# akanazawa/human_dynamics

Measured on AMD Instinct MI355X. Metric: frames/sec/GPU (ResNet+temporal+SMPL, 224x224); SMPL verts max-abs-err, higher is better.
Workload: dtype f16x3

## Files before the change

### human_dynamics_amd/_lib.py

```python
from __future__ import annotations

import ctypes as C
import os

from . import devflags

HERE = os.path.dirname(os.path.abspath(__file__))
LIB_PATH = devflags.get("LIB_PATH") or os.path.join(HERE, "libhmmr_hip.so")

HMMR_F32, HMMR_BF16, HMMR_F16X3 = 0, 1, 2
FLAG_SATURATED = 1
FLAG_NAN = 2
ABI_VERSION = 19
RESNET_UNITS = 16
RESNET_PROF_SLOTS = 64
MAX_TEMPORAL_BLOCKS = 8
MAX_REGRESSORS = 8

_vp, _fp, _ip = C.c_void_p, C.c_void_p, C.c_void_p


class ConvDesc(C.Structure):
    _fields_ = [
        ("in_", _vp), ("w", _vp), ("scale", _fp), ("shift", _fp), ("res", _vp), ("out", _vp),
        ("out2", _vp), ("scale2", _fp), ("shift2", _fp),
        ("in_dtype", C.c_int), ("out_dtype", C.c_int),
        ("n_img", C.c_int), ("hin", C.c_int), ("win", C.c_int), ("cin", C.c_int),
        ("in_img_stride", C.c_int64), ("in_row_stride", C.c_int), ("in_px_stride", C.c_int),
        ("kh", C.c_int), ("kw", C.c_int), ("sy", C.c_int), ("sx", C.c_int), ("py", C.c_int), ("px", C.c_int),
        ("ho", C.c_int), ("wo", C.c_int), ("cout", C.c_int), ("ldo", C.c_int),
        ("ldr", C.c_int), ("res_strided", C.c_int), ("res_img_stride", C.c_int64),
        ("res_row_stride", C.c_int), ("res_px_stride", C.c_int),
        ("relu", C.c_int), ("tile", C.c_int),
        ("split_k", C.c_int), ("ws", _vp), ("ws_bytes", C.c_size_t),
        ("pro_scale", _fp), ("pro_shift", _fp),
        ("out_b", _vp), ("ldo_b", C.c_int), ("n_split", C.c_int), ("relu_b", C.c_int),
        ("in2", _vp), ("cin2", C.c_int), ("k_order", C.c_int),
        ("batch", C.c_int), ("batch_in_bytes", C.c_int64), ("batch_w_bytes", C.c_int64), ("batch_out_bytes", C.c_int64),
        ("batch_res_bytes", C.c_int64), ("batch_scale_bytes", C.c_int64), ("batch_shift_bytes", C.c_int64),
    ]


class TailDesc(C.Structure):
    _fields_ = [
        ("dtype", C.c_int), ("h2", _vp), ("m", C.c_int), ("c_mid", C.c_int), ("depth", C.c_int),
        ("w3", _vp), ("scale3", _fp), ("shift3", _fp),
        ("res", _vp), ("ldr", C.c_int), ("res_strided", C.c_int), ("res_img_stride", C.c_int64),
        ("res_row_stride", C.c_int), ("res_px_stride", C.c_int), ("ho", C.c_int), ("wo", C.c_int),
        ("out", _vp), ("pre_scale", _fp), ("pre_shift", _fp),
        ("w1", _vp), ("scale1", _fp), ("shift1", _fp), ("relu1", C.c_int), ("n2", C.c_int),
        ("out_h1", _vp),
        ("h1", _vp), ("hin", C.c_int), ("win", C.c_int), ("w2", _vp), ("scale2", _fp), ("shift2", _fp),
        ("xp", _vp), ("wsc", _vp), ("shift_sc", _fp),
        ("conv2_stride", C.c_int), ("out_pre", _vp),
        ("pair_stream", _vp), ("c_xp", C.c_int), ("unit_stream", _vp), ("trunk_keep_stride", C.c_int),
    ]


class Debug(C.Structure):
    _fields_ = [("stem_route", C.c_int), ("stem_no_conv1", C.c_int), ("gemm_probe", C.c_int), ("smpl_blend_mfma", C.c_int), ("ief_no_group", C.c_int), ("reserved", C.c_int * 2), ("keep_dead_rows", C.c_int),
                ("pair_min_pixels", C.c_int), ("pair_two_tile_min", C.c_int), ("pair_form", C.c_int)]


class LaunchCounts(C.Structure):
    _fields_ = [("unit_pair", C.c_ulonglong), ("b1_unit", C.c_ulonglong), ("tail_split", C.c_ulonglong), ("conv3x3_stream", C.c_ulonglong),
                ("conv1x1_stream", C.c_ulonglong)]


class StemCounts(C.Structure):
    _fields_ = [(k, C.c_ulonglong) for k in ("fused", "fused_conv1", "repack", "gemm", "pool")]


TILE_GENERIC, TILE_PATCH, TILE_STREAM_3X3, TILE_STREAM_1X1 = range(4)
CONV_TILE_MAX = 63


class ConvTileInfo(C.Structure):
    _fields_ = [(k, C.c_int) for k in ("tile", "family", "fm", "fn", "wgm", "wgn", "pixels", "channels", "row_blocks", "depth", "occupancy", "wmax",
                                       "split_only", "conv3_form", "cols", "tune_cols", "narrow", "rank", "candidate")] + [("text", C.c_char_p)]


class Layer(C.Structure):
    _fields_ = [("w", _vp), ("scale", _fp), ("shift", _fp), ("tile", C.c_int), ("k_order", C.c_int)]


class ResnetUnit(C.Structure):
    _fields_ = [("conv1", Layer), ("conv2", Layer), ("conv3", Layer), ("shortcut", Layer), ("c3sc", Layer), ("sc_c1", Layer),
                ("w3_frag", _vp), ("w1n_frag", _vp), ("pair_stream", _vp), ("conv1_frag", _vp), ("unit_stream", _vp), ("pre_scale", _fp), ("pre_shift", _fp),
                ("c_in", C.c_int), ("base", C.c_int), ("depth", C.c_int), ("stride", C.c_int),
                ("fuse_preact", C.c_int), ("fuse_tail", C.c_int)]


class ResnetWeights(C.Structure):
    _fields_ = [("dtype", C.c_int), ("stem", Layer),
                ("unit", ResnetUnit * RESNET_UNITS), ("post_scale", _fp), ("post_shift", _fp)]


SC_NONE, SC_LAUNCH, SC_LAUNCH_WITH_CONV1, SC_IN_CONV3, SC_IN_TAIL = range(5)
CONV1_LAUNCH, CONV1_READY = range(2)
CONV2_LAUNCH, CONV2_IN_TAIL = range(2)
END_CONV3_LAUNCH, END_TAIL_BF16, END_TAIL_BF16_STRIDE2, END_TAIL_SPLIT, END_B1_UNIT, END_UNIT_PAIR = range(6)


class UnitPlan(C.Structure):
    _fields_ = [(k, C.c_int) for k in ("shortcut", "conv1", "conv2", "end", "reads_fused_preact", "writes_raw", "writes_pre",
                                       "pair_demoted", "swaps_t1_t2", "leaves_h1", "trunk_keep_stride")]


def resnet_plan(rw, n_total):
    plan = (UnitPlan * RESNET_UNITS)()
    check(load().hmmr_resnet50_plan(C.byref(rw), int(n_total), plan), "hmmr_resnet50_plan")
    return list(plan)


class TemporalBlock(C.Structure):
    _fields_ = [("gn1_gamma", _fp), ("gn1_beta", _fp), ("conv1", Layer),
                ("gn2_gamma", _fp), ("gn2_beta", _fp), ("conv2", Layer)]


class TemporalWeights(C.Structure):
    _fields_ = [("dtype", C.c_int), ("num_blocks", C.c_int), ("block", TemporalBlock * MAX_TEMPORAL_BLOCKS)]


class HallucinatorWeights(C.Structure):
    _fields_ = [("dtype", C.c_int), ("fc1", Layer), ("fc2", Layer), ("fc3", Layer)]


class IefRegressor(C.Structure):
    _fields_ = [("nd", C.c_int), ("fc1_phi", Layer), ("fc1_theta", Layer), ("fc2", Layer), ("fc3", Layer)]


class IefWeights(C.Structure):
    _fields_ = [("dtype", C.c_int), ("num_regressors", C.c_int), ("num_stages", C.c_int),
                ("reg", IefRegressor * MAX_REGRESSORS), ("mean_theta", _fp),
                ("no_optcam", C.c_int), ("delta_from_start", C.c_int)]


class IefRegGrads(C.Structure):
    _fields_ = [(k, _fp) for k in ("d_fc1_phi", "d_fc1_theta", "d_fc2", "d_fc3", "d_b1", "d_b2", "d_b3")]


class IefBwdDesc(C.Structure):
    _fields_ = [("strips", _fp), ("omega_start", _fp), ("keep", _vp), ("keep_scale", C.c_float), ("m", C.c_int), ("d_omegas", _fp),
                ("d_strips", _fp), ("d_omega_start", _fp), ("reg", IefRegGrads * MAX_REGRESSORS)]


TEMPORAL_GRAD_NAMES = ("gn1_gamma", "gn1_beta", "conv1", "b1", "gn2_gamma", "gn2_beta", "conv2", "b2")
HALLUCINATOR_GRAD_NAMES = ("fc1", "fc2", "fc3", "b1", "b2", "b3")


class TemporalBlockGrads(C.Structure):
    _fields_ = [("d_" + k, _fp) for k in TEMPORAL_GRAD_NAMES]


class TemporalBwdDesc(C.Structure):
    _fields_ = [("phi", _fp), ("b", C.c_int), ("t", C.c_int), ("d_strips", _fp), ("d_phi", _fp),
                ("block", TemporalBlockGrads * MAX_TEMPORAL_BLOCKS)]


class HallucinatorBwdDesc(C.Structure):
    _fields_ = [("phi", _fp), ("m", C.c_int), ("d_out", _fp), ("d_phi", _fp)] + [("d_" + k, _fp) for k in HALLUCINATOR_GRAD_NAMES]


DISC_POSE_LAYERS = ("conv1", "conv2", "heads", "fc1", "fc2", "fc_out")
DISC_POSE_GRAD_NAMES = ("conv1", "bc1", "conv2", "bc2", "heads", "bj", "fc1", "b1", "fc2", "b2", "fc_out", "bo")


class Rows(C.Structure):
    _fields_ = [("ptr", _fp), ("ld", C.c_int64), ("n", C.c_int)]


class DiscPoseWeights(C.Structure):
    _fields_ = [("dtype", C.c_int)] + [(k, Layer) for k in DISC_POSE_LAYERS]


class DiscPoseGrads(C.Structure):
    _fields_ = [("d_" + k, _fp) for k in DISC_POSE_GRAD_NAMES]


class DiscPoseBwdDesc(C.Structure):
    _fields_ = [("rows_a", Rows), ("rows_b", Rows), ("d_out", _fp), ("d_poses_a", _fp), ("ld_a", C.c_int64), ("d_poses_b", _fp),
                ("ld_b", C.c_int64), ("grads", DiscPoseGrads)]


class PosePriorDesc(C.Structure):
    _fields_ = [("real", Rows), ("fake", Rows), ("w_e", C.c_float), ("w_d", C.c_float), ("losses", _fp), ("d_rs_fake", _fp),
                ("grads", DiscPoseGrads)]


class SmplConsts(C.Structure):
    _fields_ = [("num_verts", C.c_int), ("num_kps", C.c_int), ("lbs_nnz", C.c_int), ("vpad", C.c_int),
                ("dirs", _fp), ("j_template", _fp), ("j_shapedirs", _fp), ("parents", _ip),
                ("lbs_idx", _ip), ("lbs_w", _fp), ("kreg_ptr", _ip), ("kreg_idx", _ip), ("kreg_val", _fp),
                ("dirs_split", _vp)]


class SmplGradConsts(C.Structure):
    _fields_ = [("num_verts", C.c_int), ("num_kps", C.c_int), ("vk_ptr", _ip), ("vk_idx", _ip), ("vk_val", _fp)]


LOSS_KP, LOSS_KP_OPTCAM, LOSS_JOINTS, LOSS_SMPL, LOSS_CONST, LOSS_SHAPE_PRIOR = 1, 2, 4, 8, 16, 32
LOSS_NAMES = ("e_kp", "e_joints", "e_smpl_pose", "e_smpl_shape", "e_const", "e_shape", "total")
LOSS_NO_VISIBLE, LOSS_NOT_FINITE = 1, 2


class SeqLossDesc(C.Structure):
    _fields_ = [("B", C.c_int), ("T", C.c_int), ("K", C.c_int), ("delta_t", C.c_int), ("flags", C.c_uint), ("weights", C.c_float * 6),
                ("kps_pred", _fp), ("joints_pred", _fp), ("rs_pred", _fp), ("beta_pred", _fp), ("ld_beta", C.c_int),
                ("kps_gt", _fp), ("joints_gt", _fp), ("rs_gt", _fp), ("shapes_gt", _fp), ("has_gt3d_smpl", _fp), ("has_gt3d_joints", _fp),
                ("losses", _fp), ("d_kps", _fp), ("d_joints", _fp), ("d_rs", _fp), ("d_beta", _fp), ("best_cam", _fp), ("status", _vp),
                ("ws", _vp), ("ws_bytes", C.c_size_t)]


# ... 266 lines not shown
```

### human_dynamics_amd/build.py

```python
from __future__ import annotations

import os
import subprocess
import sys
from concurrent.futures import ThreadPoolExecutor

HERE = os.path.dirname(os.path.abspath(__file__))
CSRC = os.path.join(HERE, "csrc")
INCLUDE = os.path.join(os.path.dirname(HERE), "include")
LIB = os.path.join(HERE, "libhmmr_hip.so")
SOURCES = ["api.cpp", "pack.cpp", "gemm_conv.hip", "conv3x3_stream.hip", "conv1x1_stream.hip", "stem.hip", "bottleneck.hip", "bottleneck_split.hip", "unit_pair.hip", "b1_unit.hip", "resnet.hip", "temporal.hip", "ief.hip", "ief_grad.hip", "movie_grad.hip", "disc_pose.hip", "smpl.hip", "smpl_grad.hip", "losses.hip", "adam.hip", "eval_metrics.hip", "preprocess.hip", "tube.hip", "track.hip", "handoff.hip", "render.hip", "collage.hip", "person_view.hip", "windows.hip", "video_plan.cpp", "video.cpp", "probe.hip"]
HIPCC = os.environ.get("HIPCC", "/opt/rocm/bin/hipcc")
FLAGS = ["--offload-arch=gfx950", "-O3", "-std=c++17", "-fPIC", "-fno-slp-vectorize", "-I", INCLUDE, "-I", CSRC,
         "-Wall", "-Wno-unused-function"]


EXTRA_FLAGS = {"pack.cpp": ["-ffp-contract=off"], "track.hip": ["-ffp-contract=off"], "collage.hip": ["-ffp-contract=off"],
               "tube.hip": ["-ffp-contract=off"], "person_view.hip": ["-ffp-contract=off"], "adam.hip": ["-ffp-contract=off"]}


def _newer(src, dst):
    return (not os.path.exists(dst)) or os.path.getmtime(src) > os.path.getmtime(dst)


def _deps():
    return sorted(os.path.join(d, h) for d in (CSRC, INCLUDE) for h in os.listdir(d) if h.endswith(".h"))


def build(force=False, verbose=True):
    objs, jobs = [], []
    for src in SOURCES:
        s = os.path.join(CSRC, src)
        o = os.path.join(CSRC, os.path.splitext(src)[0] + ".o")
        objs.append(o)
        if force or _newer(s, o) or any(_newer(d, o) for d in _deps()):
            lang = ["-x", "hip"] if src.endswith(".hip") else []
            jobs.append([HIPCC] + FLAGS + EXTRA_FLAGS.get(src, []) + lang + ["-c", s, "-o", o])

    def run(cmd):
        if verbose:
            print(" ".join(cmd), flush=True)
        r = subprocess.run(cmd, stdout=subprocess.PIPE, stderr=subprocess.STDOUT, text=True)
        if r.returncode != 0:
            raise RuntimeError("hipcc failed:\n%s\n%s" % (" ".join(cmd), r.stdout))
        if verbose and r.stdout.strip():
            print(r.stdout)

    if jobs:
        with ThreadPoolExecutor(max_workers=min(len(jobs), os.cpu_count() or 4)) as ex:
            list(ex.map(run, jobs))
    if jobs or force or not os.path.exists(LIB):
        run([HIPCC, "--offload-arch=gfx950", "-shared", "-fPIC", "-o", LIB] + objs)
        from . import isa_check
        unsafe = isa_check.unsafe_forms(LIB)
        if unsafe:
            os.replace(LIB, LIB + ".rejected")
            raise RuntimeError("the linked library holds packed-fp32 instructions gfx950 gets wrong beside MFMAs (isa_check.py, DESIGN 4.6); "
                               "kept as %s.rejected:\n%s" % (LIB, "\n".join("  %d x %s %s in %s" % (n, op, mods, kern)
                                                                             for (kern, op, mods), n in sorted(unsafe.items()))))
        if verbose:
            print("isa_check: %s" % ("no disassembler (%s) or no gfx950 code object found in the library: NOT checked" % isa_check.OBJDUMP if unsafe is None
                                     else "no packed-fp32 instruction reads source 1's high register into its low result"), flush=True)
    return LIB


if __name__ == "__main__":
    print(build(force="--force" in sys.argv))
```

### human_dynamics_amd/csrc/ief.hip

```cpp
#include "common.h"
#include "hmmr_hip.h"
#include "tail_sched.h"
#include "workspace.h"

template <typename TO>
__global__ void cast_rows_kernel(const float* __restrict__ in, TO* __restrict__ out, long long n8) {
    const long long i = (long long)blockIdx.x * blockDim.x + threadIdx.x;
    if (i >= n8) return;
    float v[8];
    load8(in + i * 8, v);
    store8(out + i * 8, v);
}

__global__ void ief_init_theta_kernel(const float* __restrict__ src, int ld_src, int off, int nd,
                                      float* __restrict__ theta, float* __restrict__ theta_other, int m, long long th_stride) {
    const long long i = (long long)blockIdx.x * blockDim.x + threadIdx.x;
    if (i >= (long long)m * LDT) return;
    const int row = (int)(i / LDT), col = (int)(i % LDT);
    const long long z = (long long)blockIdx.y * th_stride;
    theta[z + i] = col < nd ? src[(long long)row * ld_src + off + col] : 0.f;
    theta_other[z + i] = 0.f;
}

__global__ void ief_finalize_kernel(const float* __restrict__ theta, const float* __restrict__ bsrc, int ld_b,
                                    int mode, float* __restrict__ out, int m, long long th_stride) {
    const long long i = (long long)blockIdx.x * blockDim.x + threadIdx.x;
    if (i >= (long long)m * 85) return;
    const int row = (int)(i / 85), col = (int)(i % 85);
    theta += (long long)blockIdx.y * th_stride;
    out += (long long)blockIdx.y * m * 85;
    float v;
    if (mode == 0) v = theta[(long long)row * LDT + col];
    else if (col >= 75) v = bsrc[(long long)row * ld_b + col];
    else if (mode == 2) v = theta[(long long)row * LDT + col];
    else if (col == 0) v = 1.f;
    else if (col < 3) v = 0.f;
    else v = theta[(long long)row * LDT + (col - 3)];
    out[i] = v;
}

struct IefBufs { size_t xin, pre, h1, h2, th[2], sk, skbytes, pre_s, th_s, total; };
static IefBufs ief_layout(int m, int dtype, int group) {
    const size_t e = dtype == HMMR_BF16 ? 2 : 4;
    const size_t g = group > 1 ? group : 1;
    IefBufs b; WsCarver c;
    b.xin = c.take((size_t)m * 2048 * e);
    b.pre_s = align_up((size_t)m * 1024 * e, 256);
    b.th_s = align_up((size_t)m * LDT * 4, 256);
    b.pre = c.take(g * b.pre_s);
    b.h1 = c.take(g * b.pre_s);
    b.h2 = c.take(g * b.pre_s);
    b.th[0] = c.take(g * b.th_s);
    b.th[1] = c.take(g * b.th_s);
    b.skbytes = g * hmmr_conv_splitk_workspace_bytes(m, 1024, IEF_SPLIT_K);
    b.sk = c.take(b.skbytes);
    b.total = c.total();
    return b;
}

extern "C" size_t hmmr_ief_workspace_bytes(int m, int num_regressors, int dtype) {
    return m > 0 ? ief_layout(m, dtype, num_regressors - 1).total : 0;
}

extern "C" int hmmr_ief_fwd(const hmmr_ief_weights_t* w, const float* strips, int m, float* omegas,
                            void* ws, size_t ws_bytes, void* stream) {
    return hmmr_ief_fwd_from(w, strips, nullptr, m, omegas, ws, ws_bytes, stream);
}

extern "C" int hmmr_ief_fwd_from(const hmmr_ief_weights_t* w, const float* strips, const float* omega_start, int m,
                                 float* omegas, void* ws, size_t ws_bytes, void* stream) {
    HMMR_REQUIRE(w && strips && omegas && ws, "hmmr_ief_fwd: null argument");
    HMMR_REQUIRE(m > 0, "hmmr_ief_fwd: m must be positive");
    HMMR_REQUIRE(w->num_regressors >= 1 && w->num_regressors <= HMMR_MAX_REGRESSORS, "hmmr_ief_fwd: bad num_regressors");
    HMMR_REQUIRE(w->reg[0].nd == 85, "hmmr_ief_fwd: regressor 0 must predict 85-D omega");
    const int nd_delta = w->no_optcam ? 75 : 72;
    for (int r = 0; r < w->num_regressors; ++r)
        HMMR_REQUIRE(w->reg[r].nd == (r == 0 ? 85 : nd_delta), "hmmr_ief_fwd: regressor %d has nd=%d (expected %d)", r,
                     w->reg[r].nd, r == 0 ? 85 : nd_delta);
    const IefBufs L = ief_layout(m, w->dtype, w->num_regressors - 1);
    HMMR_REQUIRE(ws_bytes >= L.total, "hmmr_ief_fwd: workspace too small");
    hipStream_t s = (hipStream_t)stream;
    char* base = (char*)ws;
    const void* xin = strips;
    if (w->dtype != HMMR_F32) {
        const long long n8 = (long long)m * 2048 / 8;
        if (w->dtype == HMMR_BF16)
            hipLaunchKernelGGL(cast_rows_kernel<bf16_t>, dim3((unsigned)((n8 + 255) / 256)), dim3(256), 0, s, strips,
                               (bf16_t*)(base + L.xin), n8);
        else
            hipLaunchKernelGGL(cast_rows_kernel<bsplit_t>, dim3((unsigned)((n8 + 255) / 256)), dim3(256), 0, s, strips,
                               (bsplit_t*)(base + L.xin), n8);
        HMMR_CHECK_HIP(hipGetLastError());
        xin = base + L.xin;
    }
    void* pre = base + L.pre; void* h1 = base + L.h1; void* h2 = base + L.h2;
    float* th[2] = {(float*)(base + L.th[0]), (float*)(base + L.th[1])};
    const unsigned gth = (unsigned)(((long long)m * LDT + 255) / 256);
    const unsigned gfin = (unsigned)(((long long)m * 85 + 255) / 256);
    const int nd_group = w->num_regressors - 1;
    struct Strides { long long w, scale, shift; };
    auto strides_of = [&](const hmmr_layer_t hmmr_ief_regressor_t::*lay, Strides& st) -> bool {
        st = Strides{0, 0, 0};
        for (int r = 2; r < w->num_regressors; ++r) {
            const hmmr_layer_t& a = w->reg[r - 1].*lay; const hmmr_layer_t& b = w->reg[r].*lay;
            const Strides cur = {(const char*)b.w - (const char*)a.w,
                                 a.scale ? (const char*)b.scale - (const char*)a.scale : 0,
                                 a.shift ? (const char*)b.shift - (const char*)a.shift : 0};
            if (!a.scale != !b.scale || !a.shift != !b.shift) return false;
            if (r > 2 && (cur.w != st.w || cur.scale != st.scale || cur.shift != st.shift)) return false;
            st = cur;
        }
        return ((st.w | st.scale | st.shift) & 15) == 0;
    };
    Strides s_phi, s_th, s_fc2, s_fc3;
    const bool grouped = nd_group >= 2 && !hmmr_debug_state()->ief_no_group &&
                         strides_of(&hmmr_ief_regressor_t::fc1_phi, s_phi) && strides_of(&hmmr_ief_regressor_t::fc1_theta, s_th) &&
                         strides_of(&hmmr_ief_regressor_t::fc2, s_fc2) && strides_of(&hmmr_ief_regressor_t::fc3, s_fc3);
    const float* start = omega_start ? omega_start : w->mean_theta;
    const int ld_start = omega_start ? 85 : 0;
    const float* dsrc = w->delta_from_start ? start : (const float*)omegas;
    const int ld_d = w->delta_from_start ? ld_start : 85;
    auto run = [&](int r, int nb, const Strides& z_phi, const Strides& z_th, const Strides& z_fc2, const Strides& z_fc3) -> int {
        const hmmr_ief_regressor_t& R = w->reg[r];
        const long long ths = (long long)(L.th_s / 4);
        auto group = [&](hmmr_conv_desc_t& d, const Strides& z, long long in_b, long long out_b, long long res_b) {
            if (nb < 2) return;
            d.batch = nb; d.batch_in_bytes = in_b; d.batch_w_bytes = z.w; d.batch_out_bytes = out_b; d.batch_res_bytes = res_b;
            d.batch_scale_bytes = z.scale; d.batch_shift_bytes = z.shift;
        };
        if (r == 0)
            hipLaunchKernelGGL(ief_init_theta_kernel, dim3(gth), dim3(256), 0, s, start, ld_start, 0, 85, th[0], th[1], m, ths);
        else
            hipLaunchKernelGGL(ief_init_theta_kernel, dim3(gth, nb), dim3(256), 0, s, dsrc, ld_d, w->no_optcam ? 0 : 3, nd_delta,
                               th[0], th[1], m, ths);
        HMMR_CHECK_HIP(hipGetLastError());
        hmmr_conv_desc_t d = fc_desc(xin, w->dtype, m, 2048, R.fc1_phi, pre, w->dtype, 1024, 1024, IEF_SPLIT_K, base + L.sk, L.skbytes);
        group(d, z_phi, 0, (long long)L.pre_s, 0);
        if (hmmr_conv_gemm(&d, s)) return -2;
        int cur = 0;
        for (int st = 0; st < w->num_stages; ++st) {
            d = fc_desc(th[cur], HMMR_F32, m, LDT, R.fc1_theta, h1, w->dtype, 1024, 1024);
            d.res = pre; d.ldr = 1024; d.relu = 1;
            group(d, z_th, (long long)L.th_s, (long long)L.pre_s, (long long)L.pre_s);
            if (hmmr_conv_gemm(&d, s)) return -2;
            d = fc_desc(h1, w->dtype, m, 1024, R.fc2, h2, w->dtype, 1024, 1024, IEF_SPLIT_K, base + L.sk, L.skbytes);
            d.relu = 1;
            group(d, z_fc2, (long long)L.pre_s, (long long)L.pre_s, 0);
            if (hmmr_conv_gemm(&d, s)) return -2;
            d = fc_desc(h2, w->dtype, m, 1024, R.fc3, th[cur ^ 1], HMMR_F32, R.nd, LDT, IEF_SPLIT_K, base + L.sk, L.skbytes);
            d.res = th[cur]; d.ldr = LDT;
            group(d, z_fc3, (long long)L.pre_s, (long long)L.th_s, (long long)L.th_s);
            if (hmmr_conv_gemm(&d, s)) return -2;
            cur ^= 1;
        }
        hipLaunchKernelGGL(ief_finalize_kernel, dim3(gfin, nb), dim3(256), 0, s, (const float*)th[cur],
                           dsrc, ld_d, r == 0 ? 0 : (w->no_optcam ? 2 : 1), omegas + (size_t)r * m * 85, m, ths);
        HMMR_CHECK_HIP(hipGetLastError());
        return 0;
    };
    const Strides none = {0, 0, 0};
    if (run(0, 1, none, none, none, none)) return -2;
    if (grouped) return run(1, nd_group, s_phi, s_th, s_fc2, s_fc3);
    for (int r = 1; r < w->num_regressors; ++r)
        if (run(r, 1, none, none, none, none)) return -2;
    return 0;
}
```

### human_dynamics_amd/csrc/stream_kit.h

```cpp
#pragma once
#include <type_traits>
#include <utility>

#include "common.h"
#include "hmmr_hip.h"

template <class K, class... Args>
static int launch_with_lds(K kern, DeviceOnce& once, dim3 grid, dim3 block, int lds_attr, int lds, hipStream_t stream, Args... args) {
    if (const unsigned long long bit = once.due()) {
        HMMR_CHECK_HIP(hipFuncSetAttribute((const void*)kern, hipFuncAttributeMaxDynamicSharedMemorySize, lds_attr));
        once.mark(bit);
    }
    hipLaunchKernelGGL(kern, grid, block, lds, stream, args...);
    HMMR_CHECK_HIP(hipGetLastError());
    return 0;
}
static inline unsigned long long* probe_stamp_buffer() {
    const hmmr_debug_t* d = hmmr_debug_state();
    return (unsigned long long*)(((unsigned long long)(unsigned)d->reserved[1] << 32) | (unsigned)d->reserved[0]);
}

struct xfrag { shalf8 hi, lo; };
template <int V> using ic = std::integral_constant<int, V>;
template <class F, int... I> __device__ __forceinline__ void static_for(F&& f, std::integer_sequence<int, I...>) { (f(ic<I>{}), ...); }

typedef const __attribute__((address_space(1))) void* gptr_t;
typedef __attribute__((address_space(3))) void* lptr_t;
__device__ __forceinline__ unsigned lds_addr(void* p) { return (unsigned)(unsigned long long)(lptr_t)p; }

constexpr unsigned waitcnt_imm(int vm, int lgkm) { return (vm & 15) | (7 << 4) | (lgkm << 8) | ((vm >> 4) << 14); }
static_assert(waitcnt_imm(63, 0) == (63 | (7 << 4) | (0 << 8) | (3 << 14)) && waitcnt_imm(63, 0) == 0xC07F, "lgkmcnt(0) alone: the literal five files spelled out");
static_assert(waitcnt_imm(0, 0) == 0x0070 && waitcnt_imm(63, 15) == 0xCF7F, "everything; nothing");
static_assert(waitcnt_imm(63, 5) == 0xC57F && waitcnt_imm(37, 0) == 0x8075 && waitcnt_imm(37, 15) == 0x8F75, "lgkmcnt(5) alone; vmcnt(37) lgkmcnt(0); vmcnt(37) alone");
template <int N> __device__ __forceinline__ void wait_vm_lgkm0() {
    static_assert(N >= 0 && N < 64, "vmcnt is a 6-bit counter");
    __builtin_amdgcn_s_waitcnt(waitcnt_imm(N, 0));
}
template <int N> __device__ __forceinline__ void wait_vm() {
    static_assert(N >= 0 && N < 64, "vmcnt is a 6-bit counter");
    __builtin_amdgcn_s_waitcnt(waitcnt_imm(N, 15));
}
template <int N> __device__ __forceinline__ void wait_lgkm() {
    static_assert(N >= 0 && N <= 15, "lgkmcnt is a 4-bit counter");
    __builtin_amdgcn_s_waitcnt(waitcnt_imm(63, N));
}

template <class T, int OFF> __device__ __forceinline__ T lds_rd128(unsigned addr) {
    static_assert(sizeof(T) == 16, "a ds_read_b128");
    T v; asm volatile("ds_read_b128 %0, %1 offset:%2" : "=v"(v) : "v"(addr), "n"(OFF)); return v;
}
template <int OFF> __device__ __forceinline__ unsigned long long lds_rd64(unsigned addr) {
    unsigned long long v; asm volatile("ds_read_b64 %0, %1 offset:%2" : "=v"(v) : "v"(addr), "n"(OFF)); return v;
}
template <int OFF> __device__ __forceinline__ void lds_wr64(unsigned addr, unsigned long long v) {
    asm volatile("ds_write_b64 %0, %1 offset:%2" : : "v"(addr), "v"(v), "n"(OFF) : "memory");
}

static __device__ u32x4 g_dump_page[64 + 32] __attribute__((unused));

#ifndef TRUNK_DEAD_SHARED_PAGE
#define TRUNK_DEAD_SHARED_PAGE 0
#endif
constexpr int TRUNK_DEAD_WGS = 1024;
static __device__ u32x4 g_dead_rows[TRUNK_DEAD_WGS * 4 * 8] __attribute__((unused));
static_assert(sizeof(u32x4) * TRUNK_DEAD_WGS * 4 * 8 <= 512 * 1024, "the dead-row region lives in L2");
#define TRUNK_DEAD_ROW(wave, dlane) (TRUNK_DEAD_SHARED_PAGE ? (bsplit_t*)g_dump_page + lane * 4 \
                                     : (bsplit_t*)g_dead_rows + (((int)blockIdx.x & (TRUNK_DEAD_WGS - 1)) * 4 + (wave)) * 32 + (dlane))
static inline int trunk_keep_of(const hmmr_tail_desc_t* d) {
    const int s = hmmr_debug_state()->keep_dead_rows ? 0 : d->trunk_keep_stride;
    if (s > 1) hmmr_count_launch(HMMR_COUNT_TRUNK_KEEP);
    return s;
}
__device__ __forceinline__ unsigned trunk_live_mask(int mbase, int lane, int H, int W, int s) {
    if (s <= 1) return ~0u;
    asm volatile("" : "+s"(H), "+s"(W), "+s"(s));
    const unsigned m = (unsigned)(mbase + (lane & 31)), rem = m % (unsigned)(H * W), y = rem / (unsigned)W, x = rem - y * (unsigned)W;
    return (unsigned)__ballot(y % (unsigned)s == 0 && x % (unsigned)s == 0);
}

template <class B> __device__ __forceinline__ B stage_slot(B tile, int lr, int lh, int g, int sw, int pl) {
    return tile + lr * 128 + (((2 * g + pl) ^ sw) << 4) + 8 * lh;
}
__device__ __forceinline__ void stage_store_group(char* tile, int lr, int lh, int g, int sw, unsigned long long hi, unsigned long long lo) {
    *(unsigned long long*)stage_slot(tile, lr, lh, g, sw, 0) = hi;
    *(unsigned long long*)stage_slot(tile, lr, lh, g, sw, 1) = lo;
}
__device__ __forceinline__ void stage_store_group(char* tile, int lr, int lh, int g, int sw, const unsigned (&h)[2], const unsigned (&l)[2]) {
    *(unsigned long long*)stage_slot(tile, lr, lh, g, sw, 0) = (unsigned long long)h[0] | ((unsigned long long)h[1] << 32);
    *(unsigned long long*)stage_slot(tile, lr, lh, g, sw, 1) = (unsigned long long)l[0] | ((unsigned long long)l[1] << 32);
}
```

### human_dynamics_amd/engine.py

```python
from __future__ import annotations

import ctypes as C
import os
import threading
import time

import numpy as np
import torch

from . import _lib as L
from . import assets, devflags, packing

DTYPES = {"f32": L.HMMR_F32, "fp32": L.HMMR_F32, "float32": L.HMMR_F32,
          "bf16": L.HMMR_BF16, "bfloat16": L.HMMR_BF16,
          "f16x3": L.HMMR_F16X3, "split": L.HMMR_F16X3}
DTYPE_NAMES = {L.HMMR_F32: "f32", L.HMMR_BF16: "bf16", L.HMMR_F16X3: "f16x3"}
DEFAULT_DTYPE = "f16x3"
TILE_TABLES = os.path.join(os.path.dirname(os.path.abspath(__file__)), "tile_tables.json")


def set_debug(stem_route=0, stem_no_conv1=0, gemm_probe=0, smpl_blend_mfma=0, ief_no_group=0, pair_min_pixels=0, pair_two_tile_min=0, pair_form=0, keep_dead_rows=0):
    d = L.Debug()
    d.stem_route, d.stem_no_conv1, d.gemm_probe = int(stem_route), int(stem_no_conv1), int(gemm_probe)
    d.smpl_blend_mfma, d.ief_no_group, d.pair_min_pixels = int(smpl_blend_mfma), int(ief_no_group), int(pair_min_pixels)
    d.pair_two_tile_min, d.pair_form, d.keep_dead_rows = int(pair_two_tile_min), int(pair_form), int(keep_dead_rows)
    L.load().hmmr_set_debug(C.byref(d))


def _debug_from_env():
    e = devflags.get("STEM")
    c1 = devflags.get("STEM_C1")
    probe = int(devflags.get("GEMM_PROBE") or 0)
    if e or c1 == "0" or probe or _debug_from_env.was_set:
        set_debug(stem_route={"u": 1, "f": 2}.get(e[:1], 0), stem_no_conv1=int(c1 == "0"), gemm_probe=probe)
        _debug_from_env.was_set = bool(e or c1 == "0" or probe)


_debug_from_env.was_set = False


def _dt(d):
    if isinstance(d, str):
        if d == "bf16x3":
            import warnings
            warnings.warn("dtype 'bf16x3' is now 'f16x3' (split operands with fp16 halves since round 3)", DeprecationWarning, stacklevel=3)
            d = "f16x3"
        if d not in DTYPES:
            raise ValueError("unknown operand mode %r: use one of %s" % (d, ", ".join(sorted(set(DTYPES)))))
        return DTYPES[d]
    return int(d)


def _packer_choices(fold_sc=None, fuse_tail=None, patch_3x3=None, unit_pair=None, b1_stream=None, b1_unit=None, stem_conv1=True,
                    stream_1x1=None):
    def _flag_choice(name):
        v = devflags.get(name)
        return {"0": False, "1": True}.get(v, v)

    def pick(arg, flag):
        return flag if arg is None else arg
    fsc, fold = _flag_choice("FUSE_SC"), _flag_choice("FOLD_SC")
    return dict(fuse_preact_blocks=tuple(b for b in devflags.get("FUSE_PREACT").split(",") if b),
                fuse_tail=pick(fuse_tail, _flag_choice("FUSE_TAIL")),
                fuse_sc=fsc if isinstance(fsc, bool) else "all",
                fuse_preact_first=_flag_choice("PREACT_FIRST") is not False,
                fold_sc=pick(fold_sc, fold if isinstance(fold, bool) else None),
                patch_3x3=pick(patch_3x3, int(devflags.get("PATCH_3X3"))),
                unit_pair=pick(unit_pair, _flag_choice("UNIT_PAIR")),
                b1_stream=pick(b1_stream, _flag_choice("B1_STREAM") is True),
                b1_unit=pick(b1_unit, _flag_choice("B1_UNIT") is True),
                stem_conv1=stem_conv1,
                stream_1x1=pick(stream_1x1, _flag_choice("STREAM_1X1") is True))


class _Workspace(object):

    def __init__(self, device):
        self.device, self.buf = device, None

    def get(self, nbytes):
        if self.buf is None or self.buf.numel() < nbytes:
            self.buf = torch.empty(int(nbytes), dtype=torch.uint8, device=self.device)
        return self.buf


class HmmrEngine(object):

    def __init__(self, weights, smpl, dtype=DEFAULT_DTYPE, device="cuda:0", num_conv_layers=3,
                 delta_t_values=(-5, 5), joint_type="cocoplus", resnet_chunk=0,
                 temporal_dtype=None, ief_dtype=None, autotune=True, fold_sc=None, fuse_tail=None, patch_3x3=None,
                 unit_pair=None, b1_stream=None, b1_unit=None, stem_conv1=True, stream_1x1=None):
        self.lib = L.load()
        _debug_from_env()
        if not torch.cuda.is_available():
            raise L.HmmrError("HmmrEngine needs a HIP device (torch.cuda.is_available() is False)")
        self.device = torch.device(device)
        torch.cuda.set_device(self.device)
        self.dtype = _dt(dtype)
        self.temporal_dtype = self.dtype if temporal_dtype is None else _dt(temporal_dtype)
        self.ief_dtype = self.dtype if ief_dtype is None else _dt(ief_dtype)
        self.resnet_chunk = int(devflags.get("RESNET_CHUNK") or resnet_chunk)
        self.store = packing.DeviceStore(self.device)
        self.num_conv_layers = num_conv_layers
        self.delta_keys = sorted(int(d) for d in delta_t_values)
        w = weights if weights is not None else {}
        for name, v in w.items():
            a_ = np.asarray(v)
            if a_.dtype.kind == "f" and not np.isfinite(a_).all():
                raise ValueError("variable %r holds %d non-finite value(s)" % (name, int((~np.isfinite(a_)).sum())))
        choices = _packer_choices(fold_sc=fold_sc, fuse_tail=fuse_tail, patch_3x3=patch_3x3, unit_pair=unit_pair, b1_stream=b1_stream,
                                  b1_unit=b1_unit, stem_conv1=stem_conv1, stream_1x1=stream_1x1)
        self.rw = packing.pack_resnet(w, self.dtype, self.store, **choices) if "resnet_v2_50/conv1/weights" in w else None
        self.tw = (packing.pack_temporal(w, self.temporal_dtype, self.store, num_conv_layers)
                   if assets.temporal_scopes(0)[1] + "/weights" in w else None)
        self.hw = packing.pack_hallucinator(w, self.temporal_dtype, self.store)
        if "single_view_ief/3D_module/fc1/weights" in w and "mean_param" in w:
            self.iw, self.reg_keys = packing.pack_ief(w, self.ief_dtype, self.store, self.delta_keys)
        else:
            self.iw, self.reg_keys = None, [0]
        self._ief_source = {k: v for k, v in w.items() if k.startswith("single_view_ief") or k == "mean_param"} if self.iw is not None else None
        self._ief_bank = None
        self._movie_source = {k: v for k, v in w.items() if k.startswith(("AZ_FC_block", "fc2_res/"))} if self.tw is not None else None
        self._movie_bank = None
        self._disc_source = {k: v for k, v in w.items() if k.startswith("D_pose/")}
        self._disc_pose_bank = None
        all_f32 = (self.dtype, self.temporal_dtype, self.ief_dtype) == (L.HMMR_F32,) * 3
        self.sc = packing.pack_smpl(smpl, self.store, joint_type, split=not all_f32) if smpl is not None else None
        self._smpl_source, self.joint_type, self._gc = smpl, joint_type, None
        self.num_kps = self.sc.num_kps if self.sc is not None else assets.NUM_KPS
        self.num_verts = self.sc.num_verts if self.sc is not None else assets.NUM_VERTS
        self._ws = {k: _Workspace(self.device) for k in ("resnet", "temporal", "ief", "smpl", "hal")}
        at = devflags.get("AUTOTUNE")
        self.autotune = False if (not autotune or at == "0") else ("force" if (autotune == "force" or at == "force") else True)
        self._tiles, self._shipped = {}, set()
        self.tune_log = []
        self._tile_cache = devflags.get("TILE_CACHE")
        sources = []
        if self.autotune != "force" and devflags.get("TILE_TABLE") != "0" and os.path.exists(TILE_TABLES):
            sources.append((TILE_TABLES, True))
        if self._tile_cache and os.path.exists(self._tile_cache):
            sources.append((self._tile_cache, False))
        for path, shipped in sources:
            import json
            for key, tab in json.load(open(path)).items():
                if key.startswith("_"):
                    continue
                dt, nt = key.split(":")
                if int(dt) == self.dtype:
                    self._tiles[int(nt)] = {(int(k.split(":")[0]), k.split(":")[1]): int(v) for k, v in tab.items()}
                    if shipped:
                        self._shipped.add(int(nt))
        self.resnet_streams = int(devflags.get("RESNET_STREAMS"))
        self._side_streams = []

    @staticmethod
    def _need(packed, names):
        if packed is None:
            raise L.HmmrError("the loaded weights have no %s variables: this stage was not packed" % names)

    def _stream(self):
        return torch.cuda.current_stream(self.device).cuda_stream

    _carried_flags = {}

    def run_flags(self, clear=False):
        key = (self.device.type, self.device.index)
        v = self._device_flags(clear) | HmmrEngine._carried_flags.get(key, 0)
        if clear:
            HmmrEngine._carried_flags.pop(key, None)
        return v

    def _device_flags(self, clear):
        torch.cuda.synchronize(self.device)
        with torch.cuda.device(self.device):
            v = C.c_uint(0)
            L.check(self.lib.hmmr_run_flags(C.byref(v), int(bool(clear))), "hmmr_run_flags")
        return int(v.value)

# ... 1149 lines not shown
```

### include/hmmr_hip.h

```cpp
#ifndef HMMR_HIP_H
#define HMMR_HIP_H

#include <stddef.h>
#include <stdint.h>

#ifdef __cplusplus
extern "C" {
#endif

#define HMMR_ABI_VERSION 19

enum { HMMR_F32 = 0, HMMR_BF16 = 1, HMMR_F16X3 = 2 };

int hmmr_abi_version(void);
const char* hmmr_last_error(void);

#define HMMR_FLAG_SATURATED 1u
#define HMMR_FLAG_NAN 2u
int hmmr_run_flags(unsigned* flags, int clear);

typedef struct hmmr_debug_s {
    int stem_route;
    int stem_no_conv1;
    int gemm_probe;
    int smpl_blend_mfma;
    int ief_no_group;
    int reserved[2];
    int keep_dead_rows;
    int pair_min_pixels;
    int pair_two_tile_min;
    int pair_form;
} hmmr_debug_t;
void hmmr_set_debug(const hmmr_debug_t* d);
void hmmr_get_debug(hmmr_debug_t* d);

typedef struct {
    unsigned long long unit_pair;
    unsigned long long b1_unit;
    unsigned long long tail_split;
    unsigned long long conv3x3_stream;
    unsigned long long conv1x1_stream;
} hmmr_launch_counts_t;
void hmmr_launch_counts(hmmr_launch_counts_t* out, int clear);
unsigned long long hmmr_trunk_keep_launches(int clear);
typedef struct {
    unsigned long long fused;
    unsigned long long fused_conv1;
    unsigned long long repack;
    unsigned long long gemm;
    unsigned long long pool;
} hmmr_stem_counts_t;
void hmmr_stem_launch_counts(hmmr_stem_counts_t* out, int clear);

typedef struct {
    const void* in;
    const void* w;
    const float* scale;
    const float* shift;
    const void* res;
    void* out;
    void* out2;
    const float* scale2;
    const float* shift2;
    int in_dtype;
    int out_dtype;
    int n_img, hin, win, cin;
    int64_t in_img_stride;
    int in_row_stride, in_px_stride;
    int kh, kw, sy, sx, py, px;
    int ho, wo;
    int cout;
    int ldo;
    int ldr;
    int res_strided;
    int64_t res_img_stride;
    int res_row_stride, res_px_stride;
    int relu;
    int tile;
    int split_k;
    void* ws;
    size_t ws_bytes;
    const float* pro_scale;
    const float* pro_shift;
    void* out_b;
    int ldo_b, n_split, relu_b;
    const void* in2;
    int cin2;
    int k_order;
    int batch;
    int64_t batch_in_bytes, batch_w_bytes, batch_out_bytes, batch_res_bytes, batch_scale_bytes, batch_shift_bytes;
} hmmr_conv_desc_t;

#define HMMR_CONV_TILE_MAX 63
enum { HMMR_TILE_GENERIC = 0, HMMR_TILE_PATCH = 1, HMMR_TILE_STREAM_3X3 = 2, HMMR_TILE_STREAM_1X1 = 3 };
typedef struct {
    int tile, family;
    int fm, fn, wgm, wgn;
    int pixels, channels;
    int row_blocks;
    int depth;
    int occupancy;
    int wmax;
    int split_only;
    int conv3_form;
    int cols;
    int tune_cols;
    int narrow;
    int rank;
    int candidate;
    const char* text;
} hmmr_conv_tile_info_t;
int hmmr_conv_tile_info(int tile, hmmr_conv_tile_info_t* out);
int hmmr_conv_tile_for(int k_order, int filter_1x1, int conv3_form, int cout, int dtype, int candidate);
int hmmr_conv_tile_fits(int tile, int k_order, int filter_1x1, int conv3_form, int cout, int dtype, int win, int ksteps);
int hmmr_conv_tile_f_movie(void);

int hmmr_conv_gemm(const hmmr_conv_desc_t* d, void* stream);
size_t hmmr_conv_splitk_workspace_bytes(int m, int cout, int split_k);

typedef struct {
    const void* w;
    const float* scale;
    const float* shift;
    int tile;
    int k_order;
} hmmr_layer_t;

typedef struct {
    hmmr_layer_t conv1, conv2, conv3, shortcut;
    hmmr_layer_t c3sc;
    hmmr_layer_t sc_c1;
    const void* w3_frag;
    const void* w1n_frag;
    const void* pair_stream;
    const void* conv1_frag;
    const void* unit_stream;
    const float* pre_scale;
    const float* pre_shift;
    int c_in, base, depth, stride;
    int fuse_preact;
    int fuse_tail;
} hmmr_resnet_unit_t;

#define HMMR_RESNET_UNITS 16

typedef struct {
    int dtype;
    hmmr_layer_t stem;
    hmmr_resnet_unit_t unit[HMMR_RESNET_UNITS];
    const float* post_scale;
    const float* post_shift;
} hmmr_resnet_weights_t;

typedef struct {
    int dtype;
    const void* h2; int m; int c_mid; int depth;
    const void* w3; const float* scale3; const float* shift3;
    const void* res; int ldr; int res_strided; int64_t res_img_stride; int res_row_stride, res_px_stride; int ho, wo;
    void* out;
    const float* pre_scale; const float* pre_shift;
    const void* w1; const float* scale1; const float* shift1; int relu1; int n2;
    void* out_h1;
    const void* h1; int hin, win;
    const void* w2; const float* scale2; const float* shift2;
    const void* xp;
    const void* wsc; const float* shift_sc;
    int conv2_stride;
    void* out_pre;
    const void* pair_stream;
    int c_xp;
    const void* unit_stream;
    int trunk_keep_stride;
} hmmr_tail_desc_t;
size_t hmmr_pair_stream_bytes(int kc3, int depth, int n2);
size_t hmmr_b1_unit_stream_bytes(int c_xp);
int hmmr_mfma_rate_probe(int workgroups, int n8, float* out, void* stream);
int hmmr_clock_probe(unsigned long long* samples, int n, int sleep, const int* stop, void* stream);
size_t hmmr_conv3x3_stream_bytes(int cin, int cout);
size_t hmmr_conv1x1_stream_bytes(int cin, int cout);
int hmmr_bottleneck_tail(const hmmr_tail_desc_t* d, void* stream);
// ... 528 lines not shown
```

Baseline: 40040.

## Fuse the IEF regressor stages into one persistent LDS-resident kernel

Adds a fused IEF forward kernel. For each 16-row block it keeps the feature strips, the fc1 partial activations and theta in LDS, and runs the phi, theta, fc2 and fc3 layers for every iterative stage inside one launch with f16x3 split MFMAs. It replaces the sequence of per-layer GEMM launches, casts and theta updates when the dtype is f16x3 and m is between 256 and 512. It removes launch overhead and global round-trips of intermediates, but launches only m/16 blocks per regressor with one block per CU, so low occupancy and streaming the weights from each block are risks. A debug route field is added, reusing a reserved slot, and the probe stamp pointer is remapped so it keeps reading the same bytes.

```diff
diff --git a/human_dynamics_amd/_lib.py b/human_dynamics_amd/_lib.py
--- a/human_dynamics_amd/_lib.py
+++ b/human_dynamics_amd/_lib.py
@@ -58,7 +58,7 @@
 
 
 class Debug(C.Structure):
-    _fields_ = [("stem_route", C.c_int), ("stem_no_conv1", C.c_int), ("gemm_probe", C.c_int), ("smpl_blend_mfma", C.c_int), ("ief_no_group", C.c_int), ("reserved", C.c_int * 2), ("keep_dead_rows", C.c_int),
+    _fields_ = [("stem_route", C.c_int), ("stem_no_conv1", C.c_int), ("gemm_probe", C.c_int), ("smpl_blend_mfma", C.c_int), ("ief_no_group", C.c_int), ("ief_route", C.c_int), ("reserved", C.c_int * 1), ("keep_dead_rows", C.c_int),
                 ("pair_min_pixels", C.c_int), ("pair_two_tile_min", C.c_int), ("pair_form", C.c_int)]
 
 
diff --git a/human_dynamics_amd/build.py b/human_dynamics_amd/build.py
--- a/human_dynamics_amd/build.py
+++ b/human_dynamics_amd/build.py
@@ -9,7 +9,7 @@
 CSRC = os.path.join(HERE, "csrc")
 INCLUDE = os.path.join(os.path.dirname(HERE), "include")
 LIB = os.path.join(HERE, "libhmmr_hip.so")
-SOURCES = ["api.cpp", "pack.cpp", "gemm_conv.hip", "conv3x3_stream.hip", "conv1x1_stream.hip", "stem.hip", "bottleneck.hip", "bottleneck_split.hip", "unit_pair.hip", "b1_unit.hip", "resnet.hip", "temporal.hip", "ief.hip", "ief_grad.hip", "movie_grad.hip", "disc_pose.hip", "smpl.hip", "smpl_grad.hip", "losses.hip", "adam.hip", "eval_metrics.hip", "preprocess.hip", "tube.hip", "track.hip", "handoff.hip", "render.hip", "collage.hip", "person_view.hip", "windows.hip", "video_plan.cpp", "video.cpp", "probe.hip"]
+SOURCES = ["api.cpp", "pack.cpp", "gemm_conv.hip", "conv3x3_stream.hip", "conv1x1_stream.hip", "stem.hip", "bottleneck.hip", "bottleneck_split.hip", "unit_pair.hip", "b1_unit.hip", "resnet.hip", "temporal.hip", "ief.hip", "ief_fused.hip", "ief_grad.hip", "movie_grad.hip", "disc_pose.hip", "smpl.hip", "smpl_grad.hip", "losses.hip", "adam.hip", "eval_metrics.hip", "preprocess.hip", "tube.hip", "track.hip", "handoff.hip", "render.hip", "collage.hip", "person_view.hip", "windows.hip", "video_plan.cpp", "video.cpp", "probe.hip"]
 HIPCC = os.environ.get("HIPCC", "/opt/rocm/bin/hipcc")
 FLAGS = ["--offload-arch=gfx950", "-O3", "-std=c++17", "-fPIC", "-fno-slp-vectorize", "-I", INCLUDE, "-I", CSRC,
          "-Wall", "-Wno-unused-function"]
diff --git a/human_dynamics_amd/csrc/ief.hip b/human_dynamics_amd/csrc/ief.hip
--- a/human_dynamics_amd/csrc/ief.hip
+++ b/human_dynamics_amd/csrc/ief.hip
@@ -1,5 +1,6 @@
 #include "common.h"
 #include "hmmr_hip.h"
+#include "ief_fused.h"
 #include "tail_sched.h"
 #include "workspace.h"
 
@@ -81,6 +82,22 @@
     HMMR_REQUIRE(ws_bytes >= L.total, "hmmr_ief_fwd: workspace too small");
     hipStream_t s = (hipStream_t)stream;
     char* base = (char*)ws;
+    const float* start = omega_start ? omega_start : w->mean_theta;
+    const int ld_start = omega_start ? 85 : 0;
+    const float* dsrc = w->delta_from_start ? start : (const float*)omegas;
+    const int ld_d = w->delta_from_start ? ld_start : 85;
+    const hmmr_debug_t* dbg = hmmr_debug_state();
+    if (w->dtype == HMMR_F16X3 && !dbg->ief_no_group && dbg->ief_route != 1 &&
+        (dbg->ief_route == 2 || (m >= IEF_FUSED_M_MIN && m <= IEF_FUSED_M_MAX))) {
+        float* th0 = (float*)(base + L.th[0]);
+        const long long ths = (long long)(L.th_s / 4);
+        if (hmmr_ief_fused_launch(w, 0, 1, strips, start, ld_start, 0, nullptr, 0, 0, omegas, th0, ths, m, s)) return -2;
+        if (w->num_regressors > 1 &&
+            hmmr_ief_fused_launch(w, 1, w->num_regressors - 1, strips, dsrc, ld_d, w->no_optcam ? 0 : 3, dsrc, ld_d, w->no_optcam ? 2 : 1,
+                                  omegas, th0, ths, m, s))
+            return -2;
+        return 0;
+    }
     const void* xin = strips;
     if (w->dtype != HMMR_F32) {
         const long long n8 = (long long)m * 2048 / 8;
@@ -116,10 +133,6 @@
     const bool grouped = nd_group >= 2 && !hmmr_debug_state()->ief_no_group &&
                          strides_of(&hmmr_ief_regressor_t::fc1_phi, s_phi) && strides_of(&hmmr_ief_regressor_t::fc1_theta, s_th) &&
                          strides_of(&hmmr_ief_regressor_t::fc2, s_fc2) && strides_of(&hmmr_ief_regressor_t::fc3, s_fc3);
-    const float* start = omega_start ? omega_start : w->mean_theta;
-    const int ld_start = omega_start ? 85 : 0;
-    const float* dsrc = w->delta_from_start ? start : (const float*)omegas;
-    const int ld_d = w->delta_from_start ? ld_start : 85;
     auto run = [&](int r, int nb, const Strides& z_phi, const Strides& z_th, const Strides& z_fc2, const Strides& z_fc3) -> int {
         const hmmr_ief_regressor_t& R = w->reg[r];
         const long long ths = (long long)(L.th_s / 4);
diff --git a/human_dynamics_amd/csrc/ief_fused.h b/human_dynamics_amd/csrc/ief_fused.h
--- /dev/null
+++ b/human_dynamics_amd/csrc/ief_fused.h
@@ -0,0 +1,11 @@
+#pragma once
+#include "common.h"
+#include "hmmr_hip.h"
+
+static constexpr int IEF_FUSED_RB = 16;
+static constexpr int IEF_FUSED_M_MIN = 256;
+static constexpr int IEF_FUSED_M_MAX = 512;
+
+int hmmr_ief_fused_launch(const hmmr_ief_weights_t* w, int r0, int nb, const float* strips, const float* init_src, int ld_init,
+                          int init_off, const float* beta_src, int ld_beta, int mode, float* omegas, float* th, long long ths,
+                          int m, hipStream_t stream);
diff --git a/human_dynamics_amd/csrc/ief_fused.hip b/human_dynamics_amd/csrc/ief_fused.hip
--- /dev/null
+++ b/human_dynamics_amd/csrc/ief_fused.hip
@@ -0,0 +1,283 @@
+#include "ief_fused.h"
+#include "stream_kit.h"
+#include "tail_sched.h"
+
+namespace {
+
+constexpr int RB = IEF_FUSED_RB;
+constexpr int ROW1K = 1024 * 4 + 32;
+constexpr int ROW2K = 2048 * 4 + 32;
+constexpr int OFF_PRE = 0, OFF_H = RB * ROW1K, OFF_TH = 2 * RB * ROW1K;
+constexpr int OFF_TB = OFF_TH + RB * LDT * 4;
+constexpr int LDS_BYTES = OFF_TB + 4 * 4096;
+static_assert(RB * ROW2K <= OFF_TH, "the strips of a block lie over pre and h");
+static_assert(LDS_BYTES <= 160 * 1024, "LDS");
+
+struct FusedLayer { const void* w; const float* scale; const float* shift; };
+struct FusedReg { FusedLayer phi, th, fc2, fc3; int nd, pad_; };
+struct FusedArgs {
+    FusedReg reg[HMMR_MAX_REGRESSORS];
+    const float* strips; const float* init_src; const float* beta_src;
+    float* omegas; float* th; long long ths;
+    int ld_init, init_off, ld_beta, mode, m, stages, r0, pad_;
+};
+
+struct bfrag { u32x4 q[4]; };
+
+__device__ __forceinline__ float scale_shift(float v, const float* scale, const float* shift, int n) {
+    if (scale && shift) return fmaf(v, scale[n], shift[n]);
+    if (scale) return v * scale[n];
+    if (shift) return v + shift[n];
+    return v;
+}
+__device__ __forceinline__ int acc_row(int i, int lh) { return (i & 3) + 8 * (i >> 2) + 4 * lh; }
+
+template <int NF, int K, int DEPTH>
+__device__ __forceinline__ void split_gemm(const char* arow, const char* wbase, char* tbuf, int lane, float (&sum)[NF][8]) {
+    constexpr int NK = K / 32, KPS = NK / IEF_SPLIT_K;
+    static_assert(KPS % DEPTH == 0, "a slice is whole turns of the ring");
+    f32x16 acc[NF];
+    bfrag ring[DEPTH][NF];
+    const int srow = lane >> 3, sslot = lane & 7;
+    const char* gp = wbase + (long long)srow * (K * 4) + sslot * 16;
+    char* tw = tbuf + srow * 128;
+    const int tsw0 = (sslot ^ (srow >> 1)) << 4, tsw1 = (sslot ^ (((srow >> 1) + 4) & 7)) << 4;
+    const int flr = lane & 31, fsw = (flr >> 1) & 7, fg = (lane >> 5) * 2;
+    const char* tr = tbuf + flr * 128;
+    const int r_h0 = (fg ^ fsw) << 4, r_l0 = ((fg + 1) ^ fsw) << 4, r_h1 = ((fg + 4) ^ fsw) << 4, r_l1 = ((fg + 5) ^ fsw) << 4;
+    auto load_b = [&](bfrag (&b)[NF], int kt) {
+#pragma unroll
+        for (int f = 0; f < NF; ++f)
+#pragma unroll
+            for (int j = 0; j < 4; ++j) b[f].q[j] = *(const u32x4*)(gp + (long long)(f * 32 + j * 8) * (K * 4) + kt * 128);
+    };
+#pragma unroll
+    for (int f = 0; f < NF; ++f)
+#pragma unroll
+        for (int r = 0; r < 16; ++r) acc[f][r] = 0.f;
+#pragma unroll
+    for (int d = 0; d < DEPTH - 1; ++d) load_b(ring[d], d);
+#pragma unroll 1
+    for (int kt = 0; kt < NK; kt += DEPTH) {
+        static_for([&](auto s_) {
+            constexpr int S = decltype(s_)::value;
+            if (kt + S + DEPTH - 1 < NK) load_b(ring[(S + DEPTH - 1) % DEPTH], kt + S + DEPTH - 1);
+            __builtin_amdgcn_sched_barrier(0);
+            const char* p = arow + (kt + S) * 128;
+            const shalf8 ah0 = *(const shalf8*)p, al0 = *(const shalf8*)(p + 16);
+            const shalf8 ah1 = *(const shalf8*)(p + 64), al1 = *(const shalf8*)(p + 80);
+#pragma unroll
+            for (int f = 0; f < NF; ++f) {
+                const bfrag& b = ring[S][f];
+                *(u32x4*)(tw + tsw0) = b.q[0];
+                *(u32x4*)(tw + 1024 + tsw1) = b.q[1];
+                *(u32x4*)(tw + 2048 + tsw0) = b.q[2];
+                *(u32x4*)(tw + 3072 + tsw1) = b.q[3];
+                const shalf8 bh0 = *(const shalf8*)(tr + r_h0), bl0 = *(const shalf8*)(tr + r_l0);
+                const shalf8 bh1 = *(const shalf8*)(tr + r_h1), bl1 = *(const shalf8*)(tr + r_l1);
+                acc[f] = mfma_split(al0, bh0, acc[f]);
+                acc[f] = mfma_split(ah0, bl0, acc[f]);
+                acc[f] = mfma_split(ah0, bh0, acc[f]);
+                acc[f] = mfma_split(al1, bh1, acc[f]);
+                acc[f] = mfma_split(ah1, bl1, acc[f]);
+                acc[f] = mfma_split(ah1, bh1, acc[f]);
+            }
+        }, std::make_integer_sequence<int, DEPTH>{});
+        if ((kt + DEPTH) % KPS == 0) {
+            const bool first = kt + DEPTH == KPS;
+#pragma unroll
+            for (int f = 0; f < NF; ++f) {
+#pragma unroll
+                for (int i = 0; i < 8; ++i) sum[f][i] = first ? acc[f][i] : sum[f][i] + acc[f][i];
+#pragma unroll
+                for (int r = 0; r < 16; ++r) acc[f][r] = 0.f;
+            }
+        }
+    }
+}
+
+__device__ __forceinline__ unsigned split_cast(float v) {
+    const float c = split_clamp(v);
+    const shalf_t hi = (shalf_t)c;
+    const shalf_t lo = (shalf_t)(c - (float)hi);
+    return shalf_pack(hi, lo);
+}
+__device__ __forceinline__ unsigned split_mix(float v) {
+    const float c = split_clamp(v);
+    unsigned h, l;
+    split2_mix(c, c, h, l);
+    return (h & 0xffffu) | (l << 16);
+}
+__device__ __forceinline__ void put_split(char* base, int row, int n, unsigned hl) {
+    unsigned short* p = (unsigned short*)(base + row * ROW1K + (n >> 3) * 32 + (n & 7) * 2);
+    p[0] = (unsigned short)(hl & 0xffffu);
+    p[8] = (unsigned short)(hl >> 16);
+}
+__device__ __forceinline__ float get_split(const char* base, int row, int n) {
+    const shalf_t* p = (const shalf_t*)(base + row * ROW1K + (n >> 3) * 32 + (n & 7) * 2);
+    return (float)p[0] + (float)p[8];
+}
+
+constexpr int WIDE_NF = 2, WIDE_DEPTH = 2;
+template <int K, bool RELU>
+__device__ __forceinline__ void wide_layer(const char* arow, const FusedLayer& l, char* tbuf, int wave, int lane, int nvalid, float& satmax,
+                                           unsigned (&held)[8][8]) {
+    const int lr = lane & 31, lh = lane >> 5;
+#pragma unroll
+    for (int pass = 0; pass < 8 / WIDE_NF; ++pass) {
+        const int n0 = wave * 256 + pass * (32 * WIDE_NF);
+        float sum[WIDE_NF][8];
+        split_gemm<WIDE_NF, K, WIDE_DEPTH>(arow, (const char*)l.w + (long long)n0 * (K * 4), tbuf, lane, sum);
+#pragma unroll
+        for (int f = 0; f < WIDE_NF; ++f) {
+            const int n = n0 + f * 32 + lr;
+#pragma unroll
+            for (int i = 0; i < 8; ++i) {
+                float v = scale_shift(sum[f][i], l.scale, l.shift, n);
+                if (RELU) v = fmaxf(v, 0.f);
+                if (acc_row(i, lh) < nvalid) satmax = sat_acc(satmax, v);
+                held[pass * WIDE_NF + f][i] = split_cast(v);
+            }
+        }
+    }
+}
+__device__ __forceinline__ void put_held(char* dst, const unsigned (&held)[8][8], int wave, int lr, int lh) {
+#pragma unroll
+    for (int f = 0; f < 8; ++f)
+#pragma unroll
+        for (int i = 0; i < 8; ++i) put_split(dst, acc_row(i, lh), wave * 256 + f * 32 + lr, held[f][i]);
+}
+
+__global__ __launch_bounds__(256, 1) void ief_fused_kernel(const FusedArgs a) {
+    extern __shared__ __attribute__((aligned(16))) char smem[];
+    const int tid = threadIdx.x, lane = tid & 63;
+    const int wave = __builtin_amdgcn_readfirstlane(tid >> 6);
+    const int lr = lane & 31, lh = lane >> 5;
+    const int z = blockIdx.y;
+    const FusedReg R = a.reg[a.r0 + z];
+    const int nd = R.nd;
+    const int row0 = blockIdx.x * RB;
+    const int nvalid = min(RB, a.m - row0);
+    char* s_pre = smem + OFF_PRE;
+    char* s_h = smem + OFF_H;
+    float* s_th = (float*)(smem + OFF_TH);
+    char* tbuf = smem + OFF_TB + wave * 4096;
+    float satmax = 0.f;
+
+    for (int idx = tid; idx < RB * 256; idx += 256) {
+        const int row = idx >> 8, g = idx & 255;
+        const int srow = row0 + min(row, nvalid - 1);
+        float v[8];
+        load8(a.strips + (long long)srow * 2048 + g * 8, v);
+        store8((bsplit_t*)(smem + row * ROW2K + g * 32), v);
+    }
+    for (int idx = tid; idx < RB * LDT; idx += 256) {
+        const int row = idx / LDT, col = idx % LDT;
+        const int srow = row0 + min(row, nvalid - 1);
+        s_th[idx] = col < nd ? a.init_src[(long long)srow * a.ld_init + a.init_off + col] : 0.f;
+    }
+    __syncthreads();
+
+    const int arow_l = lr & (RB - 1);
+    unsigned held[8][8];
+    wide_layer<2048, false>(smem + arow_l * ROW2K + lh * 32, R.phi, tbuf, wave, lane, nvalid, satmax, held);
+    __syncthreads();
+    put_held(s_pre, held, wave, lr, lh);
+    __syncthreads();
+
+    for (int st = 0; st < a.stages; ++st) {
+        {
+            const float* wth = (const float*)R.th.w;
+            f32x4 bq[2][16];
+            auto load_th = [&](f32x4 (&b)[16], int fi) {
+                const float* p = wth + (long long)(wave * 256 + fi * 32 + lr) * LDT + lh * 4;
+#pragma unroll
+                for (int q = 0; q < 16; ++q) b[q] = *(const f32x4*)(p + (q >> 2) * 32 + (q & 3) * 8);
+            };
+            load_th(bq[0], 0);
+            static_for([&](auto fi_) {
+                constexpr int FI = decltype(fi_)::value;
+                if (FI + 1 < 8) load_th(bq[(FI + 1) & 1], FI + 1);
+                __builtin_amdgcn_sched_barrier(0);
+                f32x16 acc;
+#pragma unroll
+                for (int r = 0; r < 16; ++r) acc[r] = 0.f;
+                const float* ap = s_th + arow_l * LDT + lh * 4;
+#pragma unroll
+                for (int q = 0; q < 16; ++q) {
+                    const f32x4 av = *(const f32x4*)(ap + (q >> 2) * 32 + (q & 3) * 8);
+                    const f32x4 bv = bq[FI & 1][q];
+#pragma unroll
+                    for (int j = 0; j < 4; ++j) acc = __builtin_amdgcn_mfma_f32_32x32x2f32(av[j], bv[j], acc, 0, 0, 0);
+                }
+                const int n = wave * 256 + FI * 32 + lr;
+#pragma unroll
+                for (int i = 0; i < 8; ++i) {
+                    const int row = acc_row(i, lh);
+                    float v = scale_shift(acc[i], R.th.scale, R.th.shift, n);
+                    v += get_split(s_pre, row, n);
+                    v = fmaxf(v, 0.f);
+                    if (row < nvalid) satmax = sat_acc(satmax, v);
+                    put_split(s_h, row, n, split_mix(v));
+                }
+            }, std::make_integer_sequence<int, 8>{});
+        }
+        __syncthreads();
+        wide_layer<1024, true>(s_h + arow_l * ROW1K + lh * 32, R.fc2, tbuf, wave, lane, nvalid, satmax, held);
+        __syncthreads();
+        put_held(s_h, held, wave, lr, lh);
+        __syncthreads();
+        if (wave * 32 < nd) {
+            float sum[1][8];
+            split_gemm<1, 1024, 4>(s_h + arow_l * ROW1K + lh * 32, (const char*)R.fc3.w + (long long)(wave * 32) * (1024 * 4), tbuf, lane, sum);
+            const int n = wave * 32 + lr;
+            if (n < nd) {
+#pragma unroll
+                for (int i = 0; i < 8; ++i) {
+                    const int row = acc_row(i, lh);
+                    float v = scale_shift(sum[0][i], R.fc3.scale, R.fc3.shift, n);
+                    v += s_th[row * LDT + n];
+                    s_th[row * LDT + n] = v;
+                }
+            }
+        }
+        __syncthreads();
+    }
+
+    float* out = a.omegas + ((long long)z * a.m + row0) * 85;
+    for (int idx = tid; idx < nvalid * 85; idx += 256) {
+        const int row = idx / 85, col = idx % 85;
+        float v;
+        if (a.mode == 0) v = s_th[row * LDT + col];
+        else if (col >= 75) v = a.beta_src[(long long)(row0 + row) * a.ld_beta + col];
+        else if (a.mode == 2) v = s_th[row * LDT + col];
+        else if (col == 0) v = 1.f;
+        else if (col < 3) v = 0.f;
+        else v = s_th[row * LDT + (col - 3)];
+        out[idx] = v;
+    }
+    float* th = a.th + (long long)z * a.ths + (long long)row0 * LDT;
+    for (int idx = tid; idx < nvalid * LDT; idx += 256) th[idx] = s_th[idx];
+    split_flag_max(satmax);
+}
+
+}
+
+int hmmr_ief_fused_launch(const hmmr_ief_weights_t* w, int r0, int nb, const float* strips, const float* init_src, int ld_init,
+                          int init_off, const float* beta_src, int ld_beta, int mode, float* omegas, float* th, long long ths,
+                          int m, hipStream_t stream) {
+    FusedArgs a = {};
+    for (int r = 0; r < w->num_regressors; ++r) {
+        const hmmr_ief_regressor_t& g = w->reg[r];
+        a.reg[r].phi = FusedLayer{g.fc1_phi.w, g.fc1_phi.scale, g.fc1_phi.shift};
+        a.reg[r].th = FusedLayer{g.fc1_theta.w, g.fc1_theta.scale, g.fc1_theta.shift};
+        a.reg[r].fc2 = FusedLayer{g.fc2.w, g.fc2.scale, g.fc2.shift};
+        a.reg[r].fc3 = FusedLayer{g.fc3.w, g.fc3.scale, g.fc3.shift};
+        a.reg[r].nd = g.nd;
+    }
+    a.strips = strips; a.init_src = init_src; a.beta_src = beta_src; a.omegas = omegas + (size_t)r0 * m * 85; a.th = th; a.ths = ths;
+    a.ld_init = ld_init; a.init_off = init_off; a.ld_beta = ld_beta; a.mode = mode; a.m = m; a.stages = w->num_stages; a.r0 = r0;
+    static DeviceOnce once;
+    return launch_with_lds(ief_fused_kernel, once, dim3((unsigned)((m + RB - 1) / RB), (unsigned)nb), dim3(256), LDS_BYTES, LDS_BYTES,
+                           stream, a);
+}
diff --git a/human_dynamics_amd/csrc/stream_kit.h b/human_dynamics_amd/csrc/stream_kit.h
--- a/human_dynamics_amd/csrc/stream_kit.h
+++ b/human_dynamics_amd/csrc/stream_kit.h
@@ -17,7 +17,7 @@
 }
 static inline unsigned long long* probe_stamp_buffer() {
     const hmmr_debug_t* d = hmmr_debug_state();
-    return (unsigned long long*)(((unsigned long long)(unsigned)d->reserved[1] << 32) | (unsigned)d->reserved[0]);
+    return (unsigned long long*)(((unsigned long long)(unsigned)d->reserved[0] << 32) | (unsigned)d->ief_route);
 }
 
 struct xfrag { shalf8 hi, lo; };
diff --git a/human_dynamics_amd/engine.py b/human_dynamics_amd/engine.py
--- a/human_dynamics_amd/engine.py
+++ b/human_dynamics_amd/engine.py
@@ -19,11 +19,12 @@
 TILE_TABLES = os.path.join(os.path.dirname(os.path.abspath(__file__)), "tile_tables.json")
 
 
-def set_debug(stem_route=0, stem_no_conv1=0, gemm_probe=0, smpl_blend_mfma=0, ief_no_group=0, pair_min_pixels=0, pair_two_tile_min=0, pair_form=0, keep_dead_rows=0):
+def set_debug(stem_route=0, stem_no_conv1=0, gemm_probe=0, smpl_blend_mfma=0, ief_no_group=0, pair_min_pixels=0, pair_two_tile_min=0, pair_form=0, keep_dead_rows=0, ief_route=0):
     d = L.Debug()
     d.stem_route, d.stem_no_conv1, d.gemm_probe = int(stem_route), int(stem_no_conv1), int(gemm_probe)
     d.smpl_blend_mfma, d.ief_no_group, d.pair_min_pixels = int(smpl_blend_mfma), int(ief_no_group), int(pair_min_pixels)
     d.pair_two_tile_min, d.pair_form, d.keep_dead_rows = int(pair_two_tile_min), int(pair_form), int(keep_dead_rows)
+    d.ief_route = int(ief_route)
     L.load().hmmr_set_debug(C.byref(d))
 
 
diff --git a/include/hmmr_hip.h b/include/hmmr_hip.h
--- a/include/hmmr_hip.h
+++ b/include/hmmr_hip.h
@@ -25,7 +25,8 @@
     int gemm_probe;
     int smpl_blend_mfma;
     int ief_no_group;
-    int reserved[2];
+    int ief_route;
+    int reserved[1];
     int keep_dead_rows;
     int pair_min_pixels;
     int pair_two_tile_min;
```

New measurement: 39620. 0.989x the previous value.
